# huggingface/parler-tts

Hardware: NVIDIA H100
Metric: audio codec tokens/sec (all codebooks) (higher is better)
Workload: dtype bf16

## Files before the change

parler_tts_b200/csrc/step2.cu:

```cuda
#include "attn_core.cuh"
#include "common.cuh"
#include "kernels.h"
#include "ln_stats.cuh"
#include "sample_core.cuh"
#include "ptx.cuh"
#include "step.h"
#include "step_common.cuh"
#include <type_traits>

namespace ptts {
namespace cl {

constexpr int C = 2;
constexpr int V = 8;
constexpr int THREADS = 256;
constexpr int ROWS = 32;
constexpr int HROWS = 8;
constexpr int ATT_SMEM = attn_decode_smem_per_warp<bf16>();
constexpr int PROF_STRIDE = 16;
constexpr int QMAX = 6;
constexpr int OFF_STATS = 256, OFF_PART = 512, OFF_RES = 2560, OFF_CVEC = 3584;
constexpr int HDR = 5632;
constexpr int WB_BYTES = 65536;
constexpr int R_OFF = HDR + 2 * WB_BYTES;
constexpr int R_BYTES = 92160;
constexpr int QKV_OFF = R_BYTES - 2048;
constexpr int SMEM_BYTES = R_OFF + R_BYTES;
static_assert(SMEM_BYTES + 1024 <= 227 * 1024, "cluster step kernel shared memory");
static_assert(ROWS * (1024 / 2 + 8) * 2 + V * (256 + ROWS * 34 * 4) <= R_BYTES, "fc1 plan");
static_assert(HROWS * (1024 / 2 + 8) * 2 + V * C * (32 + 4 * 96 * 4) <= QKV_OFF, "QKV plan");
static_assert(5 * ATT_SMEM <= QKV_OFF && 3 * ATT_SMEM <= WB_BYTES && 16384 + 4 * 128 * 4 <= WB_BYTES, "attention plan");
static_assert(ROWS * (4096 / 4 + 8) * 2 + V * (256 + ROWS * 8 * 4) <= R_BYTES, "fc2 plan");

__device__ __forceinline__ void mbar_wait(uint64_t* bar, uint32_t parity, int what) {
  uint32_t ok, spins = 0;
  do {
    ok = mbar_try_wait_cluster(bar, parity);
    if (!ok && ++spins > (1u << 22)) { printf("ptts: cluster step mbarrier timeout (cta %d, barrier kind %d)\n", (int)blockIdx.x, what); __trap(); }
  } while (!ok);
}
__device__ __forceinline__ void st_async(uint32_t dst_cluster_addr, float v, uint32_t bar_cluster_addr) {
  asm volatile("st.async.shared::cluster.mbarrier::complete_tx::bytes.b32 [%0], %1, [%2];"
               ::"r"(dst_cluster_addr), "r"(__float_as_uint(v)), "r"(bar_cluster_addr) : "memory");
}
__device__ __forceinline__ void st_async(uint32_t dst_cluster_addr, float2 v, uint32_t bar_cluster_addr) {
  asm volatile("st.async.shared::cluster.mbarrier::complete_tx::bytes.v2.f32 [%0], {%1, %2}, [%3];"
               ::"r"(dst_cluster_addr), "f"(v.x), "f"(v.y), "r"(bar_cluster_addr) : "memory");
}
__device__ __forceinline__ uint32_t mapa(uint32_t addr, uint32_t rank) { uint32_t r; asm volatile("mapa.shared::cluster.u32 %0, %1, %2;" : "=r"(r) : "r"(addr), "r"(rank)); return r; }
__device__ __forceinline__ uint32_t cluster_rank() { uint32_t r; asm volatile("mov.u32 %0, %%cluster_ctarank;" : "=r"(r)); return r; }
__device__ __forceinline__ void cluster_arrive() { asm volatile("barrier.cluster.arrive.release.aligned;" ::: "memory"); }
__device__ __forceinline__ void cluster_wait() { asm volatile("barrier.cluster.wait.acquire.aligned;" ::: "memory"); }
__device__ __forceinline__ void cluster_arrive_reuse() { asm volatile("barrier.cluster.arrive.relaxed.aligned;" ::: "memory"); }

__host__ __device__ __forceinline__ int kslice(int kt) { return (kt & 7) >> 2; }
__host__ __device__ __forceinline__ int klocal(int kt) { return ((kt >> 3) << 2) | (kt & 3); }
__host__ __device__ __forceinline__ int kglobal(int rank, int lk) { return ((lk >> 2) << 3) | (rank << 2) | (lk & 3); }

template <int QN, int MT, bool STATS, bool ACC = false>
__device__ __forceinline__ void mma_slice(float (&out)[2][6][4], RowStatFrag& rst, const bf16* xs, int apitch, const uint4* wb, int KT, int kt0,
                                          int kt_end, int lrow, int lcol) {
  float acc[MT][QN][4];
#pragma unroll
  for (int a = 0; a < MT; a++)
#pragma unroll
    for (int j = 0; j < QN; j++)
#pragma unroll
      for (int e = 0; e < 4; e++) acc[a][j][e] = ACC ? out[a][j][e] : 0.f;
  for (int kt = kt0; kt < kt_end; kt += 4) {
    uint32_t a[MT][2][4];
#pragma unroll
    for (int mt = 0; mt < MT; mt++)
#pragma unroll
      for (int j = 0; j < 2; j++) ldmatrix_x4(a[mt][j], xs + (size_t)(mt * 16 + lrow) * apitch + kt * 32 + j * 16 + lcol);
    if (STATS) {
#pragma unroll
      for (int mt = 0; mt < MT; mt++) { row_stat_mma(rst, mt, a[mt][0]); row_stat_mma(rst, mt, a[mt][1]); }
    }
#pragma unroll
    for (int j = 0; j < QN; j++) {
      const uint4 w = wb[((size_t)j * KT + kt) * 32];
#pragma unroll
      for (int mt = 0; mt < MT; mt++) {
        mma_bf16_16816(acc[mt][j], a[mt][0], w.x, w.y);
        mma_bf16_16816(acc[mt][j], a[mt][1], w.z, w.w);
      }
    }
  }
#pragma unroll
  for (int mt = 0; mt < MT; mt++)
#pragma unroll
    for (int j = 0; j < QN; j++)
#pragma unroll
      for (int e = 0; e < 4; e++) out[mt][j][e] = acc[mt][j][e];
}

enum { PH_QKV = 0, PH_O = 1, PH_QC = 2, PH_OC = 3, PH_FC1 = 4, PH_FC2 = 5 };
constexpr int JOBS_PER_LAYER = 9;
constexpr int QKV_JOBS = 4;

__device__ __forceinline__ bool weight_job(const StepParams& p, int j, int cta, int rank, const char*& src, uint32_t& bytes) {
  const int nl = JOBS_PER_LAYER * p.L;
  if (j < nl) {
    const int l = j / JOBS_PER_LAYER, jl = j - JOBS_PER_LAYER * l;
    const int ph = jl < QKV_JOBS ? 0 : jl - (QKV_JOBS - 1);
    const int64_t idx = (ph == PH_QKV || ph == PH_QC) ? (int64_t)(cta >> 3) * C + rank : (int64_t)cta;
    const int64_t sz = p.cp_slice[ph];
    bytes = (uint32_t)(ph == PH_QKV ? sz / QKV_JOBS : sz);
    src = p.blob + p.layer0 + p.layer_stride * l + p.cp[ph] + idx * sz + (ph == PH_QKV ? jl * (sz / QKV_JOBS) : 0);
    return true;
  }
  const int task = cta + (int)gridDim.x * (j - nl);
  const int ntasks = p.K * p.V / 32;
  if (task >= ntasks) return false;
  bytes = (uint32_t)(4 * p.H * 16);
  src = p.blob + p.heads + (int64_t)task * bytes;
  return true;
}

template <int ITEMS>
__global__ void __launch_bounds__(THREADS, 1) decode_step_cluster_kernel(const __grid_constant__ StepParams p) {
  extern __shared__ __align__(128) unsigned char smem[];
  Ctrl* ctrl = p.sa.ctrl;
  if (p.prof != nullptr && blockIdx.x == 0 && threadIdx.x == 0) p.prof[(size_t)(6 * p.L + 2) * PROF_STRIDE + 3] = clock64();
  if (ctrl->active == 0) return;
  int cur_len = ctrl->cur_len;
  const unsigned gen = (unsigned)ctrl->launch_gen;
  int pos = p.P + cur_len - 1;
  const int tid = threadIdx.x, warp = tid >> 5, lane = tid & 31;
  const int H = p.H, F = p.F, B = p.B;
  const int rank = (int)cluster_rank(), peer = rank ^ 1;
  const int cta = (int)blockIdx.x;
  const int cluster = cta >> 1;
  const int head = cluster >> 2, rblk = cluster & 3;
  const int Ks = H / C, KsF = F / 4;
  const int pitch = Ks + 8, pitchF = KsF + 8;
  const int qe = F / p.nh / 64;
  const int dgrp = warp & 1, e4 = warp >> 1;

  uint64_t* abar = reinterpret_cast<uint64_t*>(smem);
  uint64_t* wbar = abar + 1;
  uint64_t* xbar = abar + 3;
  uint64_t* attbars = reinterpret_cast<uint64_t*>(smem + 128);
  float* stats = reinterpret_cast<float*>(smem + OFF_STATS);
  float* part = reinterpret_cast<float*>(smem + OFF_PART);
  float* res_s = reinterpret_cast<float*>(smem + OFF_RES);
  float* cvec = reinterpret_cast<float*>(smem + OFF_CVEC);
  unsigned char* Rg = smem + R_OFF;
  const uint32_t peer_xbar = mapa(smem_u32(xbar), (uint32_t)peer);
  uint32_t par_a = 0, par_w = 0, par_x = 0, att_parity = 0;

  if (tid == 0) {
    mbar_init<1>(abar); mbar_init<1>(&wbar[0]); mbar_init<1>(&wbar[1]); mbar_init<1>(xbar);
    asm volatile("fence.mbarrier_init.release.cluster;" ::: "memory");
  }
  attention_decode_init_warp(attbars + 2 * warp, lane);
  cluster_arrive(); cluster_wait();
  unsigned* const bar_ctr = p.bar + (gen & 1u);
  unsigned bar_target = 0u;
  if (cta == 0 && tid == 0) p.bar[(gen + 1u) & 1u] = 0u;

  const char* blob = p.blob;
  long long* const prof0 = (p.prof != nullptr && cta == 0) ? p.prof : nullptr;
  long long* prof = prof0;
  prof_mark(prof, 0);

  auto issue_weight_job = [&](int j) {
    const char* src; uint32_t bytes;
    if (!weight_job(p, j, cta, rank, src, bytes)) return;
    mbar_expect_tx(&wbar[j & 1], bytes);
    bulk_g2s_evict_first(smem + HDR + (j & 1) * WB_BYTES, src, bytes, &wbar[j & 1]);
  };
  __shared__ int s_next_active;
  const int n_steps = (p.do_sample_phase && p.n_steps > 1 && prof0 == nullptr) ? p.n_steps : 1;
  int unfinished_prev = 0;
#pragma unroll 1
  for (int it = 0; it < n_steps; it++) {
  pos = p.P + cur_len - 1;
  prof = prof0;
  cluster_arrive_reuse();
  if (tid == 0) { issue_weight_job(0); issue_weight_job(1); }

  bf16* const x_img = p.cl_x;
  bf16* const a_img = p.cl_attn;
  bf16* const h_img = p.cl_h;
  const int x_slice_elems = ROWS * pitch, h_slice_elems = ROWS * pitchF;
  auto h_offset = [&](int n) {
    const int lk = klocal(n >> 5), kq = KsF >> 5;
    return (size_t)(2 * kslice(n >> 5) + lk / kq) * h_slice_elems + (lk % kq) * 32 + (n & 31);
  };
  const int xo_slice = kslice(cta >> 2), xo_col = klocal(cta >> 2) * 32 + (cta & 3) * 8;

  {
    const int row = tid >> 3, f = tid & 7, n = cta * 8 + f;
    const float v = row < B ? embed_value(p, row, n, pos) : 0.f;
    res_s[row * 8 + f] = v;
    x_img[(size_t)xo_slice * x_slice_elems + row * pitch + xo_col + f] = __float2bfloat16_rn(v);
  }
  prof_mark(prof, 6);
  auto request_slice = [&](const bf16* img_slice, uint32_t bytes) {
    fence_proxy_async_smem();
    mbar_expect_tx(abar, bytes);
    bulk_g2s(Rg, img_slice, bytes, abar);
  };
  auto slice_of = [&](int sub, const bf16*& img, uint32_t& bytes) {
    if (sub == PH_QKV || sub == PH_QC) { img = x_img + (size_t)rank * x_slice_elems + (size_t)(HROWS * rblk) * pitch; bytes = (uint32_t)(HROWS * pitch * 2); }
    else if (sub == PH_O || sub == PH_OC) { img = a_img + (size_t)rank * x_slice_elems; bytes = (uint32_t)(x_slice_elems * 2); }
    else if (sub == PH_FC1) { img = x_img + (size_t)rank * x_slice_elems; bytes = (uint32_t)(x_slice_elems * 2); }
    else { img = h_img + (size_t)(2 * rank) * h_slice_elems; bytes = (uint32_t)(h_slice_elems * 2); }
  };
  {
    const bf16* nimg; uint32_t nbytes;
    slice_of(PH_QKV, nimg, nbytes);
    bar_target = grid_sync(bar_ctr, bar_target, -1, false, nullptr, [&]() { request_slice(nimg, nbytes); });
  }
  prof_mark(prof, 7);

  const int lrow = (lane & 7) + ((lane >> 3) & 1) * 8, lcol = (lane >> 4) * 8;
  const int g = lane >> 2, t4 = lane & 3;
  const int n_phases = 6 * p.L;

  const int att_row = HROWS * rblk + 4 * rank + (warp >> 1);
  const int att_slice = kslice(2 * head), att_col = klocal(2 * head) * 32;

#pragma unroll 1
  for (int ph = 0; ph < n_phases; ph++) {
    const int l = ph / 6, sub = ph - 6 * l;
    prof = prof0 ? prof0 + (size_t)(ph + 1) * PROF_STRIDE : nullptr;
    prof_mark(prof, 0);
    const char* lb = blob + p.layer0 + p.layer_stride * l;
    const bool rowpart = (sub == PH_QKV || sub == PH_QC);
    const bool has_ln = (sub == PH_QKV || sub == PH_QC || sub == PH_FC1);
    const int q = (sub == PH_QKV) ? 6 : (sub == PH_QC ? 2 : (sub == PH_FC1 ? qe : 1));
    const int Nc = 4 * q * 8;
    const int KT = (sub == PH_FC2 ? KsF : Ks) >> 5;
    const int apitch = (sub == PH_FC2) ? pitchF : pitch;
    const int act_bytes = (rowpart ? HROWS : ROWS) * apitch * 2;
    const int RS = (q == 1) ? 8 : 8 * q + 2;
    const int blk = rowpart ? 32 + 4 * 16 * q * 4 : 256 + ROWS * RS * 4;
    unsigned char* const recv = Rg + ((act_bytes + 127) & ~127);
    const uint32_t peer_recv = mapa(smem_u32(recv), (uint32_t)peer);
    const uint32_t xbytes = 4u * (rowpart ? V * 4 * 16 * q + V / 2 * 4 * 2 : V / C * (ROWS * 8 * q + (has_ln ? ROWS * 2 : 0)));
    auto put = [&](int d, uint32_t off, auto v) {
      if (d == rank) *reinterpret_cast<decltype(v)*>(recv + off) = v;
      else st_async(peer_recv + off, v, peer_xbar);
    };
    const int j0 = JOBS_PER_LAYER * l + (sub == 0 ? 0 : sub + QKV_JOBS - 1);
    if (tid == 0) mbar_expect_tx(xbar, xbytes);

    float cv1 = 0.f, cv2 = 0.f;
    if (has_ln) {
      const float* c1; int ntot;
      if (sub == PH_QKV) { c1 = reinterpret_cast<const float*>(lb + p.c_qkv); ntot = p.qkv_rows; }
      else if (sub == PH_QC) { c1 = reinterpret_cast<const float*>(lb + p.c_qc); ntot = H; }
      else { c1 = reinterpret_cast<const float*>(lb + p.c_fc1); ntot = F; }
      const int nown = rowpart ? Nc : 8 * q;
      if (tid < nown) {
        int n;
        if (sub == PH_QKV) n = (tid >> 6) * (p.nh * HD) + head * HD + (tid & 63);
        else if (sub == PH_QC) n = head * HD + tid;
        else n = cta * 8 * q + tid;
        cv1 = c1[n];
        cv2 = c1[ntot + n];
      }
    }

    auto wait_job = [&](int j) {
      mbar_wait(&wbar[j & 1], (par_w >> (j & 1)) & 1u, 1);
      par_w ^= 1u << (j & 1);
    };
    auto ring = [&](int j) { return reinterpret_cast<const uint4*>(smem + HDR + (j & 1) * WB_BYTES) + lane; };
    wait_job(j0);
    if (sub == PH_QKV) wait_job(j0 + 1);
    mbar_wait(abar, par_a, 0);
    par_a ^= 1u;
    prof_mark(prof, 1);
    float acc[2][QMAX][4];
    RowStatFrag rst;
    row_stat_zero(rst);
    {
      const bf16* xs = reinterpret_cast<const bf16*>(Rg);
      if (rowpart) {
        auto head_pass = [&](auto pass_tag) {
          constexpr int P = decltype(pass_tag)::value;
          const int u = 2 * P + dgrp;
          float t[2][QMAX][4];
          if (sub == PH_QKV) mma_slice<6, 1, P == 0>(t, rst, xs, apitch, ring(j0 + u), KT, e4, KT, lrow & 7, lcol);
          else mma_slice<2, 1, P == 0>(t, rst, xs, apitch, ring(j0) + (size_t)(2 * u) * KT * 32, KT, e4, KT, lrow & 7, lcol);
          const int d = g >> 2;
          const uint32_t slot = (uint32_t)((8 * rank + warp) * blk);
          if (P == 0) {
            cluster_wait();
            if (dgrp == 0) {
              const uint32_t so = slot + 8 * (g & 3);
              if (t4 == 0) put(d, so, rst.s1[0][0]);
              if (t4 == (g >> 1)) put(d, so + 4, (g & 1) ? rst.sq[0][0][1] : rst.sq[0][0][0]);
            }
          }
#pragma unroll
          for (int j = 0; j < QMAX; j++)
            if (j < q) put(d, slot + 32 + 4 * ((g & 3) * 16 * q + P * 8 * q + j * 8 + 2 * t4), make_float2(t[0][j][0], t[0][j][1]));
        };
        head_pass(std::integral_constant<int, 0>{});
        if (sub == PH_QKV) {
          prof_mark(prof, 8);
          __syncthreads();
          if (tid == 0) { issue_weight_job(j0 + 2); issue_weight_job(j0 + 3); }
          wait_job(j0 + 2);
          wait_job(j0 + 3);
          prof_mark(prof, 9);
        }
        head_pass(std::integral_constant<int, 1>{});
      } else if (sub == PH_FC2) {
        auto quarter = [&](auto qq_tag) {
          constexpr int QQ = decltype(qq_tag)::value;
          const uint4* wq = ring(j0) + (size_t)dgrp * 2 * KT * 32 + (size_t)QQ * KT * 32;
          mma_slice<1, 2, false, QQ == 1>(acc, rst, xs, apitch, wq, 2 * KT, (e4 - QQ * KT) & 3, KT, lrow, lcol);
        };
        quarter(std::integral_constant<int, 0>{});
        prof_mark(prof, 8);
        __syncthreads();
        if (tid == 0) request_slice(h_img + (size_t)(2 * rank + 1) * h_slice_elems, (uint32_t)(h_slice_elems * 2));
        mbar_wait(abar, par_a, 0);
        par_a ^= 1u;
        prof_mark(prof, 9);
        quarter(std::integral_constant<int, 1>{});
      } else {
        const uint4* wb = ring(j0) + (size_t)(dgrp * q) * KT * 32;
        if (sub == PH_FC1) {
          if (q == 4) mma_slice<4, 2, true>(acc, rst, xs, apitch, wb, KT, e4, KT, lrow, lcol);
          else if (q == 2) mma_slice<2, 2, true>(acc, rst, xs, apitch, wb, KT, e4, KT, lrow, lcol);
          else mma_slice<1, 2, true>(acc, rst, xs, apitch, wb, KT, e4, KT, lrow, lcol);
        } else mma_slice<1, 2, false>(acc, rst, xs, apitch, wb, KT, e4, KT, lrow, lcol);
      }
    }
    prof_mark(prof, 2);
    prof_mark(prof, 12);
    if (!rowpart) cluster_wait();
    prof_mark(prof, 13);
    if (!rowpart) {
      const uint32_t slot = (uint32_t)((4 * rank + e4) * blk);
#pragma unroll
      for (int mt = 0; mt < 2; mt++)
#pragma unroll
        for (int j = 0; j < QMAX; j++) {
          if (j < q) {
            const uint32_t o = slot + 256 + 4 * ((mt * 16 + g) * RS + j * 8 + 2 * t4);
            put(dgrp, o, make_float2(acc[mt][j][0], acc[mt][j][1]));
            put(dgrp, o + 4 * 8 * RS, make_float2(acc[mt][j][2], acc[mt][j][3]));
          }
        }
      if (has_ln) {
#pragma unroll
        for (int mt = 0; mt < 2; mt++) {
          const uint32_t s0 = slot + 8 * (mt * 16 + g), s8 = s0 + 8 * 8;
          if (t4 == 0) { put(dgrp, s0, rst.s1[mt][0]); put(dgrp, s8, rst.s1[mt][2]); }
          if (t4 == (g >> 1)) {
            put(dgrp, s0 + 4, (g & 1) ? rst.sq[mt][0][1] : rst.sq[mt][0][0]);
            put(dgrp, s8 + 4, (g & 1) ? rst.sq[mt][1][3] : rst.sq[mt][1][2]);
          }
        }
      }
    }
    prof_mark(prof, 14);
    if (has_ln && tid < (rowpart ? Nc : 8 * q)) { cvec[tid] = cv1; cvec[256 + tid] = cv2; }
    __syncthreads();
    if (warp == 1 && lane == 0 && !rowpart && sub != PH_OC) issue_weight_job(j0 + 2);
    if (warp == 1 && lane == 0 && sub == PH_QKV) issue_weight_job(j0 + QKV_JOBS);
    prof_mark(prof, 15);
    mbar_wait(xbar, par_x, 2);
    par_x ^= 1u;
    prof_mark(prof, 3);

    if (!rowpart) {
      const int row = tid >> 3, f0 = tid & 7;
      float ln_mean = 0.f, ln_rstd = 0.f;
      if (has_ln) {
        float S1 = 0.f, S2 = 0.f;
#pragma unroll
        for (int v = 0; v < V; v++) { const float2 x = *reinterpret_cast<const float2*>(recv + (size_t)v * blk + row * 8); S1 += x.x; S2 += x.y; }
        ln_mean = S1 / (float)H;
        ln_rstd = rsqrtf(fmaxf(S2 / (float)H - ln_mean * ln_mean, 0.f) + p.eps);
      }
      if (row < B && sub == PH_FC1 && q == 4) {
        const int f = 4 * f0;
        float v[4] = {0.f, 0.f, 0.f, 0.f};
#pragma unroll
        for (int sv = 0; sv < V; sv++) {
          const float* bp = reinterpret_cast<const float*>(recv + (size_t)sv * blk + 256) + row * RS + f;
          const float2 a = *reinterpret_cast<const float2*>(bp), b2 = *reinterpret_cast<const float2*>(bp + 2);
          v[0] += a.x; v[1] += a.y; v[2] += b2.x; v[3] += b2.y;
        }
#pragma unroll
        for (int e = 0; e < 4; e++) v[e] = apply_act(DT<bf16>::rnd(ln_rstd * (v[e] - ln_mean * cvec[f + e]) + cvec[256 + f + e]), p.act);
        uint2 pk;
        pk.x = att_pack(v[0], v[1]); pk.y = att_pack(v[2], v[3]);
        *reinterpret_cast<uint2*>(h_img + h_offset(cta * 32 + f) + row * pitchF) = pk;
      } else if (row < B) {
        for (int i = 0; i < q; i++) {
          const int f = f0 + 8 * i;
          float v = 0.f;
#pragma unroll
          for (int sv = 0; sv < V; sv++) v += reinterpret_cast<const float*>(recv + (size_t)sv * blk + 256)[row * RS + f];
          if (sub == PH_FC1) {
            v = ln_rstd * (v - ln_mean * cvec[f]) + cvec[256 + f];
            v = apply_act(DT<bf16>::rnd(v), p.act);
            h_img[h_offset(cta * 8 * q + f) + row * pitchF] = __float2bfloat16_rn(v);
          } else {
            v = DT<bf16>::rnd(res_s[row * 8 + f] + DT<bf16>::rnd(v));
            res_s[row * 8 + f] = v;
            x_img[(size_t)xo_slice * x_slice_elems + row * pitch + xo_col + f] = __float2bfloat16_rn(v);
          }
        }
      }
    } else {
      bf16* qkv_s = reinterpret_cast<bf16*>(Rg + QKV_OFF);
      auto gather = [&](auto jw_tag) {
        constexpr int JW = decltype(jw_tag)::value, NC = 4 * JW, QCW = 2 * JW;
        for (int idx = tid; idx < 4 * NC; idx += THREADS) {
          const int r4 = idx / NC, col = idx - r4 * NC;
          const int u = col / JW, cw = (u >> 1) * JW + (col - u * JW);
          float S1 = 0.f, S2 = 0.f;
#pragma unroll
          for (int e = 0; e < V; e++) {
            const float2 x = *reinterpret_cast<const float2*>(recv + (size_t)(8 * (e >> 2) + 2 * (e & 3)) * blk + r4 * 8);
            S1 += x.x; S2 += x.y;
          }
          const float ln_mean = S1 / (float)H;
          const float ln_rstd = rsqrtf(fmaxf(S2 / (float)H - ln_mean * ln_mean, 0.f) + p.eps);
          float v = 0.f;
#pragma unroll
          for (int e = 0; e < V; e++)
            v += reinterpret_cast<const float*>(recv + (size_t)(8 * (e >> 2) + 2 * (e & 3) + (u & 1)) * blk + 32)[r4 * QCW + cw];
          v = ln_rstd * (v - ln_mean * cvec[col]) + cvec[256 + col];
          qkv_s[idx] = __float2bfloat16_rn(v);
        }
      };
      if (sub == PH_QKV) gather(std::integral_constant<int, 48>{}); else gather(std::integral_constant<int, 16>{});
      static_assert(HD == 64, "QKV: 2 x 2 units of 6 n-tiles (q|k|v of a head), q_cross: 2 x 2 units of 2 n-tiles");
    }
    prof_mark(prof, 4);
    __syncthreads();
    cluster_arrive_reuse();

    if (rowpart) {
      if (att_row < B) {
        AttnArgs att = decode_attn_args(p, l, pos, sub == PH_QC);
        const bf16* qkv_s = reinterpret_cast<const bf16*>(Rg + QKV_OFF);
        const int row_base = HROWS * rblk + 4 * rank;
        const bf16* qbase = qkv_s - (size_t)row_base * Nc - (size_t)head * HD;
        att.q = qbase; att.ldq = Nc;
        att.ldo = pitch;
        att.out = a_img + (size_t)att_slice * x_slice_elems + att_col - (size_t)head * HD;
        if (sub == PH_QKV) { att.knew = qbase; att.vnew = qbase; att.ldkv = Nc; att.k_col0 = HD; att.v_col0 = 2 * HD; }
        unsigned char* wb0 = smem + HDR;
        unsigned char* held = wb0 + ((sub == PH_QKV ? j0 + 1 : j0) & 1) * WB_BYTES;
        unsigned char* other = wb0 + ((sub == PH_QKV ? j0 : j0 + 1) & 1) * WB_BYTES;
        unsigned char* region = warp < 5 ? Rg + (size_t)warp * ATT_SMEM : held + (size_t)(warp - 5) * ATT_SMEM;
        float* xr = reinterpret_cast<float*>(other + 16384) + (warp >> 1) * 128;
        attention_decode_item_warp<bf16>(att, att_row, head, pos, region, attbars + 2 * warp, lane, att_parity, warp & 1, 2, xr, (warp >> 1) + 1);
      }
      prof_mark(prof, 5);
    }
    prof_mark(prof, 6);
    if (p.prof != nullptr && l == p.L / 2 && tid == 0) {
      unsigned long long ns;
      asm volatile("mov.u64 %0, %%globaltimer;" : "=l"(ns));
      p.prof[(size_t)(n_phases + 4) * PROF_STRIDE + sub * (int)gridDim.x + cta] = (long long)ns;
    }

    const bool last = (ph + 1 == n_phases);
    const bf16* nimg; uint32_t nbytes;
    if (last) { nimg = x_img; nbytes = (uint32_t)(C * x_slice_elems * 2); }
    else slice_of((sub + 1) % 6, nimg, nbytes);
    const int held_job = sub == PH_QKV ? j0 + QKV_JOBS + 1 : (sub == PH_QC || sub == PH_OC) ? j0 + 2 : -1;
    bar_target = grid_sync(bar_ctr, bar_target, ph, false, nullptr, [&]() {
      request_slice(nimg, nbytes);
      if (held_job >= 0) issue_weight_job(held_job);
    });
    prof_mark(prof, 7);
  }
  cluster_wait();

  prof = prof0 ? prof0 + (size_t)(n_phases + 1) * PROF_STRIDE : nullptr;
  prof_mark(prof, 0);
  {
    const int ntasks = p.K * p.V / 32;
    const float* c1 = reinterpret_cast<const float*>(blob + p.c_heads);
    const float* c2 = c1 + p.K * p.V;
    mbar_wait(abar, par_a, 3);
    par_a ^= 1u;
    const bf16* xs = reinterpret_cast<const bf16*>(Rg);
    const int KTH = H >> 5;
    auto ktile = [&](int kt) { return xs + (size_t)kslice(kt) * x_slice_elems + klocal(kt) * 32; };
    {
      RowStatFrag rst;
      row_stat_zero(rst);
      for (int kt = warp; kt < KTH; kt += 8) {
        const bf16* sl = ktile(kt);
#pragma unroll
        for (int mt = 0; mt < 2; mt++)
#pragma unroll
          for (int j = 0; j < 2; j++) {
            uint32_t a[4];
            ldmatrix_x4(a, sl + (size_t)(mt * 16 + lrow) * pitch + j * 16 + lcol);
            row_stat_mma(rst, mt, a);
          }
      }
      row_stat_store(rst, part, warp, lane);
      __syncthreads();
      row_stat_finalize(part, H, ROWS, p.eps, stats);
      __syncthreads();
    }
    prof_mark(prof, 1);
    constexpr int HRS = 40;
    int job = JOBS_PER_LAYER * p.L;
    for (int task = cta; task < ntasks; task += (int)gridDim.x, job++) {
      mbar_wait(&wbar[job & 1], (par_w >> (job & 1)) & 1u, 4);
      par_w ^= 1u << (job & 1);
      float acc[2][4][4];
#pragma unroll
      for (int a = 0; a < 2; a++)
#pragma unroll
        for (int j = 0; j < 4; j++)
#pragma unroll
          for (int e = 0; e < 4; e++) acc[a][j][e] = 0.f;
      unsigned char* wbuf = smem + HDR + (job & 1) * WB_BYTES;
      const uint4* wb = reinterpret_cast<const uint4*>(wbuf) + lane;
      for (int kt = warp; kt < KTH; kt += 8) {
        const bf16* sl = ktile(kt);
        uint32_t a[2][2][4];
#pragma unroll
        for (int mt = 0; mt < 2; mt++)
#pragma unroll
          for (int j = 0; j < 2; j++) ldmatrix_x4(a[mt][j], sl + (size_t)(mt * 16 + lrow) * pitch + j * 16 + lcol);
#pragma unroll
        for (int j = 0; j < 4; j++) {
          const uint4 w = wb[((size_t)j * KTH + kt) * 32];
#pragma unroll
          for (int mt = 0; mt < 2; mt++) {
            mma_bf16_16816(acc[mt][j], a[mt][0], w.x, w.y);
            mma_bf16_16816(acc[mt][j], a[mt][1], w.z, w.w);
          }
        }
      }
      __syncthreads();
      float* red = reinterpret_cast<float*>(wbuf);
#pragma unroll
      for (int mt = 0; mt < 2; mt++)
#pragma unroll
        for (int j = 0; j < 4; j++) {
          float* base = red + ((size_t)warp * 32 + mt * 16 + g) * HRS + j * 8 + 2 * t4;
          *reinterpret_cast<float2*>(base) = make_float2(acc[mt][j][0], acc[mt][j][1]);
          *reinterpret_cast<float2*>(base + 8 * HRS) = make_float2(acc[mt][j][2], acc[mt][j][3]);
        }
      __syncthreads();
      {
        const int er = tid >> 3, ec = tid & 7;
        if (er < B) {
          const float mean = stats[2 * er], rstd = stats[2 * er + 1];
#pragma unroll
          for (int j = 0; j < 4; j++) {
            const int cidx = j * 8 + ec, n = task * 32 + cidx;
            float v = 0.f;
#pragma unroll
            for (int w = 0; w < 8; w++) v += red[((size_t)w * 32 + er) * HRS + cidx];
            p.logits[(size_t)er * p.K * p.V + n] = DT<bf16>::rnd(rstd * (v - mean * c1[n]) + c2[n]);
          }
        }
      }
      __syncthreads();
      if (tid == 32) {
        fence_proxy_async_smem();
        issue_weight_job(job + 2);
      }
    }
  }
  prof_mark(prof, 6);
  bar_target = grid_sync(bar_ctr, bar_target, n_phases, true);
  prof = prof0 ? prof0 + (size_t)(n_phases + 2) * PROF_STRIDE : nullptr;
  prof_mark(prof, 0);
  if (p.do_sample_phase) {
    const ptts_gen_params gp = *p.sa.gen;
    const int BK = B * p.K;
    sample_phase<ITEMS>(p.sa, gp, BK, cur_len);
    prof_mark(prof, 1);
    bar_target = grid_sync(bar_ctr, bar_target, n_phases + 1, true, nullptr, [&]() {
      const int tot = *reinterpret_cast<volatile int*>(&ctrl->n_unfinished);
      s_next_active = (tot - unfinished_prev > 0) ? 1 : 0;
      unfinished_prev = tot;
    });
    prof_mark(prof, 2);
  }
  bool go_on = false;
  if (p.do_sample_phase) {
    const int act = s_next_active;
    if (cta == 0 && tid == 0) {
      ctrl->cur_len = cur_len + 1;
      ctrl->active = act;
      ctrl->steps_run += 1;
    }
    go_on = act != 0;
    cur_len += 1;
  }
  if (!go_on) break;
  }
  if (cta == 0 && tid == 0) {
    if (p.do_sample_phase) ctrl->n_unfinished = 0;
    ctrl->launch_gen = (int)(gen + 1u);
  }
}

__global__ void cluster_pack_kernel(const uint4* __restrict__ src, uint4* __restrict__ dst, int ph, int nh, int ntc, int kts, int KT_src) {
  const int64_t tile = blockIdx.x;
  const int ktl = (int)(tile % kts);
  const int j = (int)((tile / kts) % ntc);
  const int slice = (int)(tile / ((int64_t)kts * ntc));
  const int rank = slice & 1, owner = slice >> 1;
  int n_tile;
  if (ph == PH_QKV) n_tile = (j >> 3) * (nh * 8) + owner * 8 + (j & 7);
  else n_tile = owner * ntc + j;
  const int kt = kglobal(rank, ktl);
  dst[tile * 32 + threadIdx.x] = src[((int64_t)n_tile * KT_src + kt) * 32 + threadIdx.x];
}

}

int cluster_pack_layer(const char* layer_src, char* layer_dst, const int64_t* mat_off, const int64_t* cp_off, int nh, int H, int F, cudaStream_t st) {
  const int ks = H / cl::C / 32, ksf = F / cl::C / 32;
  const int ntc[6] = {24, 2, 8, 2, F / (4 * nh) / 8, 2};
  const int owners[6] = {nh, 4 * nh, nh, 4 * nh, 4 * nh, 4 * nh};
  for (int ph = 0; ph < 6; ph++) {
    const int kts = (ph == 5) ? ksf : ks;
    const int KT_src = (ph == 5) ? F / 32 : H / 32;
    const int64_t tiles = (int64_t)owners[ph] * cl::C * ntc[ph] * kts;
    cl::cluster_pack_kernel<<<(unsigned)tiles, 32, 0, st>>>(reinterpret_cast<const uint4*>(layer_src + mat_off[ph]),
                                                            reinterpret_cast<uint4*>(layer_dst + cp_off[ph]), ph, nh, ntc[ph], kts, KT_src);
  }
  PTTS_LAUNCH_CHECK();
  return PTTS_OK;
}

static const void* cluster_kernel_fn(const StepParams& p) {
  if (p.sample_items <= 1) return (const void*)cl::decode_step_cluster_kernel<1>;
  if (p.sample_items <= 5) return (const void*)cl::decode_step_cluster_kernel<5>;
  return (const void*)cl::decode_step_cluster_kernel<9>;
}

static void cluster_launch_config(const StepParams& p, cudaLaunchConfig_t& cfg, cudaLaunchAttribute* at, cudaStream_t st) {
  cfg = cudaLaunchConfig_t{};
  cfg.gridDim = dim3((unsigned)(4 * p.nh * cl::C));
  cfg.blockDim = dim3(cl::THREADS);
  cfg.dynamicSmemBytes = cl::SMEM_BYTES;
  cfg.stream = st;
  at[0].id = cudaLaunchAttributeClusterDimension;
  at[0].val.clusterDim.x = cl::C; at[0].val.clusterDim.y = 1; at[0].val.clusterDim.z = 1;
  at[1].id = cudaLaunchAttributeCooperative;
  at[1].val.cooperative = 1;
  cfg.attrs = at;
  cfg.numAttrs = 2;
}

bool cluster_step_available(const StepParams& p) {
  const void* fn = cluster_kernel_fn(p);
  static bool told = false;
  auto why = [&](const char* what, cudaError_t e, int n) {
    if (!told) fprintf(stderr, "ptts_b200: cluster step kernel not used (%s: %s, %d co-resident clusters of %d, need %d); the one-CTA-per-SM step kernel runs instead\n",
                       what, cudaGetErrorString(e), n, cl::C, 4 * p.nh);
    told = true;
    cudaGetLastError();
    return false;
  };
  cudaError_t e = cudaFuncSetAttribute(fn, cudaFuncAttributeMaxDynamicSharedMemorySize, cl::SMEM_BYTES);
  if (e != cudaSuccess) return why("shared memory attribute", e, 0);
  cudaLaunchConfig_t cfg; cudaLaunchAttribute at[2];
  cluster_launch_config(p, cfg, at, nullptr);
  cfg.numAttrs = 1;
  int n = 0;
  e = cudaOccupancyMaxActiveClusters(&n, fn, &cfg);
  if (e != cudaSuccess) return why("cluster occupancy query", e, n);
  if (n < 4 * p.nh) return why("too few co-resident clusters", cudaSuccess, n);
  return true;
}

int launch_decode_step_cluster(const StepParams& p, cudaStream_t st) {
  const void* fn = cluster_kernel_fn(p);
  cudaLaunchConfig_t cfg; cudaLaunchAttribute at[2];
  cluster_launch_config(p, cfg, at, st);
  void* args[] = {(void*)&p};
  PTTS_CHECK_CUDA(cudaLaunchKernelExC(&cfg, fn, args));
  return PTTS_OK;
}

}
```

Baseline: 237,500.

## Prefetch QKV second-pass weights early into spare smem to overlap with compute

The second half of the QKV weights was previously fetched only after the first head pass, behind a full block barrier and wait. Most of those weights are now bulk-loaded during the preceding grid sync, into a new region of the R buffer and the unused tails of the weight ring buffers, tracked by two new mbarriers. The remaining sixth is issued after a 128-thread named barrier once the ring slot is free. This hides weight-load latency at the cost of more shared memory, a more intricate split of the work across warps, and parity bookkeeping.

```diff
diff --git a/parler_tts_b200/csrc/step2.cu b/parler_tts_b200/csrc/step2.cu
--- a/parler_tts_b200/csrc/step2.cu
+++ b/parler_tts_b200/csrc/step2.cu
@@ -23,12 +23,12 @@
 constexpr int HDR = 5632;
 constexpr int WB_BYTES = 65536;
 constexpr int R_OFF = HDR + 2 * WB_BYTES;
-constexpr int R_BYTES = 92160;
+constexpr int R_BYTES = 93184;
 constexpr int QKV_OFF = R_BYTES - 2048;
 constexpr int SMEM_BYTES = R_OFF + R_BYTES;
 static_assert(SMEM_BYTES + 1024 <= 227 * 1024, "cluster step kernel shared memory");
 static_assert(ROWS * (1024 / 2 + 8) * 2 + V * (256 + ROWS * 34 * 4) <= R_BYTES, "fc1 plan");
-static_assert(HROWS * (1024 / 2 + 8) * 2 + V * C * (32 + 4 * 96 * 4) <= QKV_OFF, "QKV plan");
+static_assert(HROWS * (1024 / 2 + 8) * 2 + V * C * (32 + 4 * 96 * 4) + 7 * 16 * 512 <= QKV_OFF, "QKV plan");
 static_assert(5 * ATT_SMEM <= QKV_OFF && 3 * ATT_SMEM <= WB_BYTES && 16384 + 4 * 128 * 4 <= WB_BYTES, "attention plan");
 static_assert(ROWS * (4096 / 4 + 8) * 2 + V * (256 + ROWS * 8 * 4) <= R_BYTES, "fc2 plan");
 
@@ -57,7 +57,7 @@
 __host__ __device__ __forceinline__ int klocal(int kt) { return ((kt >> 3) << 2) | (kt & 3); }
 __host__ __device__ __forceinline__ int kglobal(int rank, int lk) { return ((lk >> 2) << 3) | (rank << 2) | (lk & 3); }
 
-template <int QN, int MT, bool STATS, bool ACC = false>
+template <int QN, int MT, bool STATS, bool ACC = false, int J0 = 0>
 __device__ __forceinline__ void mma_slice(float (&out)[2][6][4], RowStatFrag& rst, const bf16* xs, int apitch, const uint4* wb, int KT, int kt0,
                                           int kt_end, int lrow, int lcol) {
   float acc[MT][QN][4];
@@ -66,7 +66,7 @@
 #pragma unroll
     for (int j = 0; j < QN; j++)
 #pragma unroll
-      for (int e = 0; e < 4; e++) acc[a][j][e] = ACC ? out[a][j][e] : 0.f;
+      for (int e = 0; e < 4; e++) acc[a][j][e] = ACC ? out[a][J0 + j][e] : 0.f;
   for (int kt = kt0; kt < kt_end; kt += 4) {
     uint32_t a[MT][2][4];
 #pragma unroll
@@ -92,7 +92,7 @@
 #pragma unroll
     for (int j = 0; j < QN; j++)
 #pragma unroll
-      for (int e = 0; e < 4; e++) out[mt][j][e] = acc[mt][j][e];
+      for (int e = 0; e < 4; e++) out[mt][J0 + j][e] = acc[mt][j][e];
 }
 
 enum { PH_QKV = 0, PH_O = 1, PH_QC = 2, PH_OC = 3, PH_FC1 = 4, PH_FC2 = 5 };
@@ -141,6 +141,7 @@
   uint64_t* abar = reinterpret_cast<uint64_t*>(smem);
   uint64_t* wbar = abar + 1;
   uint64_t* xbar = abar + 3;
+  uint64_t* qbar = abar + 4;
   uint64_t* attbars = reinterpret_cast<uint64_t*>(smem + 128);
   float* stats = reinterpret_cast<float*>(smem + OFF_STATS);
   float* part = reinterpret_cast<float*>(smem + OFF_PART);
@@ -148,10 +149,10 @@
   float* cvec = reinterpret_cast<float*>(smem + OFF_CVEC);
   unsigned char* Rg = smem + R_OFF;
   const uint32_t peer_xbar = mapa(smem_u32(xbar), (uint32_t)peer);
-  uint32_t par_a = 0, par_w = 0, par_x = 0, att_parity = 0;
+  uint32_t par_a = 0, par_w = 0, par_x = 0, par_q = 0, att_parity = 0;
 
   if (tid == 0) {
-    mbar_init<1>(abar); mbar_init<1>(&wbar[0]); mbar_init<1>(&wbar[1]); mbar_init<1>(xbar);
+    mbar_init<1>(abar); mbar_init<1>(&wbar[0]); mbar_init<1>(&wbar[1]); mbar_init<1>(xbar); mbar_init<1>(&qbar[0]); mbar_init<1>(&qbar[1]);
     asm volatile("fence.mbarrier_init.release.cluster;" ::: "memory");
   }
   attention_decode_init_warp(attbars + 2 * warp, lane);
@@ -170,6 +171,27 @@
     if (!weight_job(p, j, cta, rank, src, bytes)) return;
     mbar_expect_tx(&wbar[j & 1], bytes);
     bulk_g2s_evict_first(smem + HDR + (j & 1) * WB_BYTES, src, bytes, &wbar[j & 1]);
+  };
+  const uint32_t qkv_r_off = (((uint32_t)(HROWS * pitch * 2) + 127u) & ~127u) + 16u * (32u + 4u * 16u * 6u * 4u);
+  auto issue_qkv_pass1 = [&](int jq) {
+    const char *s2, *s3; uint32_t b;
+    weight_job(p, jq + 2, cta, rank, s2, b);
+    weight_job(p, jq + 3, cta, rank, s3, b);
+    const uint32_t nt = b / 6;
+    unsigned char* ra = smem + HDR + (jq & 1) * WB_BYTES;
+    unsigned char* rb = smem + HDR + ((jq + 1) & 1) * WB_BYTES;
+    mbar_expect_tx(&qbar[0], 11u * nt);
+    bulk_g2s_evict_first(Rg + qkv_r_off, s2, 5u * nt, &qbar[0]);
+    bulk_g2s_evict_first(Rg + qkv_r_off + 5u * nt, s3, 2u * nt, &qbar[0]);
+    bulk_g2s_evict_first(ra + b, s3 + 2u * nt, 2u * nt, &qbar[0]);
+    bulk_g2s_evict_first(rb + b, s3 + 4u * nt, 2u * nt, &qbar[0]);
+  };
+  auto issue_qkv_pass1_late = [&](int jq) {
+    const char* s2; uint32_t b;
+    weight_job(p, jq + 2, cta, rank, s2, b);
+    const uint32_t nt = b / 6;
+    mbar_expect_tx(&qbar[1], nt);
+    bulk_g2s_evict_first(smem + HDR + (jq & 1) * WB_BYTES, s2 + 5u * nt, nt, &qbar[1]);
   };
   __shared__ int s_next_active;
   const int n_steps = (p.do_sample_phase && p.n_steps > 1 && prof0 == nullptr) ? p.n_steps : 1;
@@ -212,7 +234,7 @@
   {
     const bf16* nimg; uint32_t nbytes;
     slice_of(PH_QKV, nimg, nbytes);
-    bar_target = grid_sync(bar_ctr, bar_target, -1, false, nullptr, [&]() { request_slice(nimg, nbytes); });
+    bar_target = grid_sync(bar_ctr, bar_target, -1, false, nullptr, [&]() { request_slice(nimg, nbytes); issue_qkv_pass1(0); });
   }
   prof_mark(prof, 7);
 
@@ -285,8 +307,22 @@
           constexpr int P = decltype(pass_tag)::value;
           const int u = 2 * P + dgrp;
           float t[2][QMAX][4];
-          if (sub == PH_QKV) mma_slice<6, 1, P == 0>(t, rst, xs, apitch, ring(j0 + u), KT, e4, KT, lrow & 7, lcol);
-          else mma_slice<2, 1, P == 0>(t, rst, xs, apitch, ring(j0) + (size_t)(2 * u) * KT * 32, KT, e4, KT, lrow & 7, lcol);
+          if (sub == PH_QKV && P == 0) mma_slice<6, 1, true>(t, rst, xs, apitch, ring(j0 + u), KT, e4, KT, lrow & 7, lcol);
+          else if (sub == PH_QKV) {
+            const uint4* rq = reinterpret_cast<const uint4*>(Rg + qkv_r_off) + lane;
+            const size_t nt = (size_t)KT * 32;
+            if (dgrp == 0) {
+              mma_slice<5, 1, false>(t, rst, xs, apitch, rq, KT, e4, KT, lrow & 7, lcol);
+              prof_mark(prof, 10);
+              mbar_wait(&qbar[1], par_q, 6);
+              prof_mark(prof, 11);
+              mma_slice<1, 1, false, false, 5>(t, rst, xs, apitch, ring(j0), KT, e4, KT, lrow & 7, lcol);
+            } else {
+              mma_slice<2, 1, false>(t, rst, xs, apitch, rq + 5 * nt, KT, e4, KT, lrow & 7, lcol);
+              mma_slice<2, 1, false, false, 2>(t, rst, xs, apitch, ring(j0) + 6 * nt, KT, e4, KT, lrow & 7, lcol);
+              mma_slice<2, 1, false, false, 4>(t, rst, xs, apitch, ring(j0 + 1) + 6 * nt, KT, e4, KT, lrow & 7, lcol);
+            }
+          } else mma_slice<2, 1, P == 0>(t, rst, xs, apitch, ring(j0) + (size_t)(2 * u) * KT * 32, KT, e4, KT, lrow & 7, lcol);
           const int d = g >> 2;
           const uint32_t slot = (uint32_t)((8 * rank + warp) * blk);
           if (P == 0) {
@@ -304,13 +340,15 @@
         head_pass(std::integral_constant<int, 0>{});
         if (sub == PH_QKV) {
           prof_mark(prof, 8);
-          __syncthreads();
-          if (tid == 0) { issue_weight_job(j0 + 2); issue_weight_job(j0 + 3); }
-          wait_job(j0 + 2);
-          wait_job(j0 + 3);
+          if (dgrp == 0) {
+            asm volatile("bar.sync 5, 128;" ::: "memory");
+            if (tid == 0) issue_qkv_pass1_late(j0);
+          }
+          mbar_wait(&qbar[0], par_q, 5);
           prof_mark(prof, 9);
         }
         head_pass(std::integral_constant<int, 1>{});
+        if (sub == PH_QKV) par_q ^= 1u;
       } else if (sub == PH_FC2) {
         auto quarter = [&](auto qq_tag) {
           constexpr int QQ = decltype(qq_tag)::value;
@@ -477,6 +515,7 @@
     bar_target = grid_sync(bar_ctr, bar_target, ph, false, nullptr, [&]() {
       request_slice(nimg, nbytes);
       if (held_job >= 0) issue_weight_job(held_job);
+      if (sub == PH_FC2 && !last) issue_qkv_pass1(j0 + 1);
     });
     prof_mark(prof, 7);
   }
```

Result: faster. 245,400 (median of 6 runs) (+3.3%).
